# shaunlebron/blinky

Measured on AMD Instinct MI355X. Metric: warped Mpixels/s (lensmap apply), higher is better.
Workload: dtype u8; 1 GPU; 3840x2160 cube/panini f_fov 180, 64 frames/step from a resident ring of 64 distinct globes (1.80 GB, advanced every step), one lensmap; value / ms_per_step = the job with steps alternating between 2 HIP stream(s), value_one_stream = the same on one stream, roofline.kernel_ms_per_launch = the kernel alone under HIP events; 64 frames/step since r5 (r1-r4 ran 16: compare those with value_at_16_frames; ring_globes=64, parallelism=row-stripes x1, streams=2

## Files before the change

### blinky_amd/csrc/bk_api.cpp

```cpp
#include "bk_internal.h"

#include <algorithm>
#include <cstdlib>
#include <cstring>
#include <ctime>
#include <vector>

#include <dlfcn.h>

static thread_local std::string g_create_error;

static bool g_hwq_late = false;
__attribute__((constructor)) static void bk_more_hardware_queues()
{
    const char *keep = getenv("BLINKY_HIP_KEEP_HW_QUEUES");
    if (keep && *keep && *keep != '0') return;
    if (getenv("GPU_MAX_HW_QUEUES")) return;
    if (void *h = dlopen("libamdhip64.so", RTLD_NOW | RTLD_NOLOAD)) { g_hwq_late = true; (void)dlclose(h); }
    (void)setenv("GPU_MAX_HW_QUEUES", "16", 0);
}
void bk::hw_queue_note()
{
    static bool said = false;
    if (said) return;
// ... 320 lines not shown
    return BK_OK;
}

bk::DebugOptions bk::g_debug;
#if BK_DEBUG_API
extern "C" int bk_debug_set_option(const char *name, int value)
{
    if (!name) return BK_E_INVALID;
    if (!strcmp(name, "no_memcache")) bk::g_debug.no_memcache = value;
    else if (!strcmp(name, "libm_rel_log2")) bk::g_debug.libm_rel_log2 = value;
    else if (!strcmp(name, "print_model")) bk::g_debug.print_model = value;
    else if (!strcmp(name, "host_module")) bk::g_debug.host_module = value;
    else if (!strcmp(name, "no_direct_submit")) bk::g_debug.no_direct_submit = value;
    else if (!strcmp(name, "forward_careful")) bk::g_debug.forward_careful = value;
    else return BK_E_INVALID;
    return BK_OK;
}
#endif
#if BK_DEBUG_API
extern "C" int bk_debug_set_ablation(bk_ctx *ctx, int bits)
{
    if (!ctx) return BK_E_INVALID;
    ctx->apply_flags = bits;
    return BK_OK;
}
#endif

#if BK_DEBUG_API
extern "C" int bk_debug_set_tile_shape(bk_ctx *ctx, int lw)
{
    if (!ctx) return BK_E_INVALID;
    if (lw >= 600) { ctx->apply_block_cost = lw == 600 ? -1 : lw - 601; bk::coopmap_invalidate(ctx); return BK_OK; }
    if (lw >= 400) { ctx->apply_lds_kb = lw - 400; bk::coopmap_invalidate(ctx); return BK_OK; }
    if (lw >= 300) { ctx->apply_fchunk = lw - 300; return BK_OK; }
    if (lw >= 100) { ctx->apply_wgs_per_cu = lw - 100; return BK_OK; }
    if (lw != 0 && lw != 1 && lw != 2 && lw != 4) return BK_E_INVALID;
    ctx->tile_shape = lw;
    bk::coopmap_invalidate(ctx);
    return BK_OK;
}
#endif

#if BK_DEBUG_API
extern "C" int bk_debug_tile_stats(bk_ctx *ctx, int out[6])
{
    if (!ctx || !out) return BK_E_INVALID;
    if (!ctx->lensmap_valid) return ctx->fail(BK_E_STATE, "no lensmap");
    if (int r = ensure_device(ctx)) return r;
    return bk::coopmap_stats(ctx, out);
}
#endif

#if BK_DEBUG_API
extern "C" int bk_debug_traffic_model(bk_ctx *ctx, uint64_t out[8])
{
    if (!ctx || !out) return BK_E_INVALID;
    if (!ctx->lensmap_valid) return ctx->fail(BK_E_STATE, "no lensmap");
    if (int r = ensure_device(ctx)) return r;
    return bk::coopmap_traffic_model(ctx, out);
}
#endif

#if BK_DEBUG_API
extern "C" int bk_debug_band_balance(bk_ctx *ctx, uint32_t out[18])
{
    if (!ctx || !out) return BK_E_INVALID;
    if (!ctx->lensmap_valid) return ctx->fail(BK_E_STATE, "no lensmap");
    if (int r = ensure_device(ctx)) return r;
    return bk::coopmap_band_balance(ctx, out);
}
#endif

#if BK_DEBUG_API
extern "C" int bk_debug_xcd_of_workgroups(bk_ctx *ctx, int *out, int nworkgroups)
{
    if (!ctx || !out || nworkgroups < 1) return BK_E_INVALID;
    if (int r = ensure_device(ctx)) return r;
    return bk::coopmap_xcd_probe(ctx, out, nworkgroups);
}
#endif

extern "C" double bk_last_build_ms(const bk_ctx *ctx) { return ctx ? ctx->last_build_ms : 0; }


extern "C" int bk_set_lensmap(bk_ctx *ctx, const uint32_t *offsets, const uint8_t *tints)
{
    if (!ctx || !offsets) return BK_E_INVALID;
    if (!ctx->d_offsets) return ctx->fail(BK_E_STATE, "bk_set_lensmap: call bk_resize first");
    if (int r = ensure_device(ctx)) return r;
    const size_t px = (size_t)ctx->W * ctx->rows();
    BK_HIP(ctx, hipMemcpyAsync(ctx->d_offsets, offsets, px * 4, hipMemcpyHostToDevice, ctx->stream));
    if (int r = bk::launch_convert_offsets(ctx, ctx->d_offsets, px, 1)) return r;
    if (tints) BK_HIP(ctx, hipMemcpyAsync(ctx->d_tints, tints, px, hipMemcpyHostToDevice, ctx->stream));
    else BK_HIP(ctx, hipMemsetAsync(ctx->d_tints, 255, px, ctx->stream));
    if (int r = bk::subtexel_alloc(ctx)) return r;
    if (ctx->d_subtexel) BK_HIP(ctx, hipMemsetAsync(ctx->d_subtexel, 0x80, px * 2, ctx->stream));
    BK_HIP(ctx, hipStreamSynchronize(ctx->stream));
    bk::lensmap_replaced(ctx);
    return BK_OK;
}

int bk::subtexel_alloc(bk_ctx *ctx)
{
    if (!ctx->subtexel_on || ctx->d_subtexel || !ctx->map_px) return BK_OK;
    BK_HIP(ctx, hipMalloc((void **)&ctx->d_subtexel, ctx->map_px * sizeof(uint16_t)));
    return BK_OK;
// ... 940 lines not shown
```

### blinky_amd/csrc/bk_apply_coop.hip

```cpp
#include <algorithm>
#include <cmath>
#include <cstdio>
#include <cstdlib>
#include <cstring>
#include <ctime>
#include <vector>

#include "bk_internal.h"
#include "bk_resident_plan.h"

namespace bk {

constexpr int BK_PAL_BYTES = BK_MAX_PLATES * 256;
constexpr int BK_COOP_MAX_FLIPS = 4;
constexpr int BK_COOP_LDS_CAP = 65536;
constexpr uint32_t BK_COOP_MAX_CHUNKS = 4095;
constexpr uint32_t CF_ALL = 0x1, CF_NONE = 0x10;
constexpr uint32_t CF_SLOW = 0x100, CF_EMPTY = 0x200;
constexpr uint32_t BK_COOP_BINS = 65;
constexpr int BK_COOP_STATS = 208;
constexpr int BK_COOP_BLOCK_COST = 4;

enum BkAblation : int {
    BK_AB_NO_GLOBE_LOADS = 2,
// ... 21 lines not shown
constexpr int BK_KF_ALIGNED4 = 1024;
constexpr int BK_KF_ALIGNED16 = 2048;
constexpr int BK_KF_DIRECT = 1 << 27;
constexpr int BK_KF_WGMAP = 1 << 30;
static_assert((BK_RF_KERNEL_MASK & (BK_KF_ALIGNED4 | BK_KF_ALIGNED16)) == 0, "a developer bit would read as a frame alignment in the resident kernel");
static_assert((int)BK_RF_NO_STORES == (int)BK_AB_NO_STORES, "coop_gather_store reads one no-stores bit for the batch and the resident kernel");

constexpr int CS_MAX_CHUNKS = 0;
constexpr int CS_SLOW_BLOCKS = 1;
constexpr int CS_EMPTY_BLOCKS = 2;
constexpr int CS_LINES = 3;
constexpr int CS_CHUNKS = 4;
constexpr int CS_UNEVEN_BANDS = 7;
constexpr int CS_HIST_BLOCKS = 8;
constexpr int CS_HIST_LINES = CS_HIST_BLOCKS + BK_COOP_BINS;
constexpr int CS_HIST_CHUNKS = CS_HIST_LINES + BK_COOP_BINS;
static_assert(CS_HIST_CHUNKS + (int)BK_COOP_BINS <= BK_COOP_STATS, "a statistics replica holds the three histograms");

struct CoopHdr {
    uint32_t nchunks;
    uint32_t flags;
};

struct CoopMap {
    CoopHdr *d_hdr = nullptr;
    uint32_t *d_list = nullptr;
    uint16_t *d_idx = nullptr;
    bool tinted = false;
    uint32_t *d_cost = nullptr;
    uint32_t *d_order = nullptr;
    uint32_t *d_cum = nullptr;
    uint32_t *d_bands = nullptr;
    uint32_t *d_wgmap = nullptr;
    uint32_t *d_stats = nullptr;
    int blocks_x = 0, blocks_y = 0;
    int rg = 4;
    int lds_bytes = 0;
    int tuned_frames = 0;
    int single_form = 0;
    int fchunk = 0;
    bool lds_fixed = false;
    struct Tuned { int rg = 0, kb = 0, form = 0, fchunk = 0, frames = 0; } tuned[3];
    int flips = 0;
    int grown_rg = 0;
    uint32_t stats[BK_COOP_STATS] = {0};
    uint32_t *h_stats = nullptr;
    hipEvent_t stats_ready = nullptr;
    bool stats_pending = false;
    int slow_blocks = 0;
    bool valid = false;
    size_t alloc_px = 0, alloc_blocks = 0;
};

template <int RG>
__global__ __launch_bounds__(256) void coop_compile_kernel(const uint32_t *__restrict__ lmap, const uint8_t *__restrict__ tints,
                                                           int W, int rows, int blocks_x, int nblocks,
                                                           CoopHdr *__restrict__ hdr, uint32_t *__restrict__ list,
                                                           uint16_t *__restrict__ idx, int tinted,
                                                           uint32_t *__restrict__ stats, int row_stride, uint32_t *__restrict__ cost,
                                                           int block_cost)
{
    constexpr int NP = 4 * RG, N = 256 * NP;
    __shared__ uint32_t key[N];
    __shared__ uint32_t uniq[N];
    __shared__ uint32_t s_wsum[4], s_wlines[4], s_wpx[4];
    __shared__ uint32_t s_flags;
    const int lane = threadIdx.x & 63, wave = threadIdx.x >> 6;
    const bool survey = row_stride > 1;
    const int sby = blockIdx.x / blocks_x, bx = blockIdx.x - sby * blocks_x;
    const int by = sby * row_stride, blk = by * blocks_x + bx;
    constexpr int LPR = 32 / RG;
    const int oy = by * 8 * RG;
    const int ry = wave * 2 * RG + lane / LPR;
    const int x0 = bx * 128 + (lane % LPR) * 4 * RG;
    if (threadIdx.x == 0) s_flags = 0;

    uint32_t o[NP];
    uint32_t kc[NP];
    bool all_l = true, any_l = false;
    uint32_t npx = 0;
#pragma unroll
    for (int i = 0; i < NP; ++i) {
        const int row = oy + ry, x = x0 + i;
        const bool in = row < rows && x < W;
        o[i] = in ? lmap[(size_t)row * W + x] : BK_NULL_OFFSET;
        const uint32_t tn = in && tinted ? tints[(size_t)row * W + x] : 255u;
        kc[i] = o[i] == BK_NULL_OFFSET ? 0xFFFFFFFFu : ((o[i] >> 4) << 3) | (tn < (uint32_t)BK_MAX_PLATES ? tn + 1u : 0u);
        key[threadIdx.x * NP + i] = kc[i];
        all_l = all_l && o[i] != BK_NULL_OFFSET;
        any_l = any_l || o[i] != BK_NULL_OFFSET;
        npx += o[i] != BK_NULL_OFFSET ? 1u : 0u;
    }
    const bool all = __all(all_l), any = __any(any_l);
    __syncthreads();
    if (lane == 0) atomicOr(&s_flags, (all ? CF_ALL << wave : 0u) | (any ? 0u : CF_NONE << wave));

    for (int k = 2; k <= N; k <<= 1) {
        for (int j = k >> 1; j > 0; j >>= 1) {
            for (int t = threadIdx.x; t < N / 2; t += 256) {
                const int i = ((t & ~(j - 1)) << 1) | (t & (j - 1)), p = i | j;
                const uint32_t a = key[i], b = key[p];
                const bool up = (i & k) == 0;
                if ((a > b) == up) { key[i] = b; key[p] = a; }
            }
            __syncthreads();
        }
    }

    uint32_t cnt = 0, lcnt = 0;
#pragma unroll
    for (int i = 0; i < NP; ++i) {
        const int p = threadIdx.x * NP + i;
        const uint32_t v = key[p], prev = p > 0 ? key[p - 1] : 0xFFFFFFFFu;
        const bool first = v != 0xFFFFFFFFu && (p == 0 || v != prev);
        cnt += first ? 1u : 0u;
        lcnt += (first && (p == 0 || (v >> 6) != (prev >> 6))) ? 1u : 0u;
    }
    uint32_t incl = cnt, lsum = lcnt;
    for (int m = 1; m < 64; m <<= 1) {
        const uint32_t u = __shfl_up(incl, m);
        if (lane >= m) incl += u;
    }
    for (int m = 32; m >= 1; m >>= 1) { lsum += __shfl_xor(lsum, m); npx += __shfl_xor(npx, m); }
    if (lane == 63) s_wsum[wave] = incl;
    if (lane == 0) { s_wlines[wave] = lsum; s_wpx[wave] = npx; }
    __syncthreads();
    uint32_t base = incl - cnt;
    for (int w = 0; w < wave; ++w) base += s_wsum[w];
    const uint32_t nchunks = s_wsum[0] + s_wsum[1] + s_wsum[2] + s_wsum[3];
    const uint32_t lines = s_wlines[0] + s_wlines[1] + s_wlines[2] + s_wlines[3];
    const uint32_t mapped = s_wpx[0] + s_wpx[1] + s_wpx[2] + s_wpx[3];
    const bool slow = nchunks > BK_COOP_MAX_CHUNKS;
    {
        uint32_t k = base;
#pragma unroll
        for (int i = 0; i < NP; ++i) {
            const int p = threadIdx.x * NP + i;
            const uint32_t v = key[p];
            if (v != 0xFFFFFFFFu && (p == 0 || v != key[p - 1])) {
                uniq[k] = v;
                if (!slow && !survey) list[(size_t)blk * N + k] = ((v >> 3) << 4) | (v & 7u);
                ++k;
            }
        }
    }
    __syncthreads();

    if (!survey) {
#pragma unroll
    for (int r = 0; r < RG; ++r) {
        uint32_t a[4];
#pragma unroll
        for (int k = 0; k < 4; ++k) {
            const int i = r * 4 + k;
            a[k] = 0xFFFFu;
            if (o[i] != BK_NULL_OFFSET) {
                a[k] = 0;
                if (!slow) {
                    const uint32_t c = kc[i];
                    uint32_t lo = 0, hi = nchunks;
                    while (lo < hi) {
                        const uint32_t mid = (lo + hi) >> 1;
                        if (uniq[mid] < c) lo = mid + 1; else hi = mid;
                    }
                    a[k] = lo * 16u + (o[i] & 15u);
                }
            }
        }
        const size_t slab = (((size_t)blk * 4 + wave) * RG + r) * 256 + (size_t)lane * 4;
        *reinterpret_cast<uint2 *>(idx + slab) = make_uint2(a[0] | (a[1] << 16), a[2] | (a[3] << 16));
    }
    }
    if (threadIdx.x == 0) {
        const uint32_t wflags = s_flags;
        const bool any_blk = nchunks != 0;
        CoopHdr h;
        h.nchunks = slow ? 0u : nchunks;
        h.flags = wflags | (slow ? CF_SLOW : 0u) | (any_blk ? 0u : CF_EMPTY);
        if (!survey) {
            hdr[blk] = h;
            cost[blk] = !any_blk ? 0u : slow ? (uint32_t)N / 4u : lines + mapped * 5u / 512u + (uint32_t)block_cost;
        }
        uint32_t *st = stats + (blk & 63) * BK_COOP_STATS;
        if (!slow && any_blk) {
            atomicMax(&st[CS_MAX_CHUNKS], nchunks);
            const uint32_t bin = min(BK_COOP_BINS - 1u, (nchunks * 16u + 1023u) / 1024u);
            atomicAdd(&st[CS_HIST_BLOCKS + bin], 1u);
            atomicAdd(&st[CS_HIST_LINES + bin], lines);
            atomicAdd(&st[CS_HIST_CHUNKS + bin], nchunks);
            atomicAdd(&st[CS_LINES], lines);
            atomicAdd(&st[CS_CHUNKS], nchunks);
        }
        if (slow) atomicAdd(&st[CS_SLOW_BLOCKS], 1u);
        if (!any_blk) atomicAdd(&st[CS_EMPTY_BLOCKS], 1u);
    }
}

#define BK_LDS_BARRIER()                                                           \
    do {                                                                           \
        if (kflags & BK_AB_SYNCTHREADS) __syncthreads();                           \
        else asm volatile("s_waitcnt lgkmcnt(0)\n\ts_barrier" ::: "memory");       \
    } while (0)

template <int RG>
struct CoopIdx {
    uint2 iw[RG];
};
__device__ __forceinline__ uint4 bk_tint_chunk(uint4 q, uint32_t e, const uint8_t *pal_s)
{
    const uint32_t cls = e & 7u;
    if (cls) {
        const uint8_t *row = pal_s + (cls - 1u) * 256u;
        uint32_t w[4] = {q.x, q.y, q.z, q.w};
#pragma unroll
        for (int i = 0; i < 4; ++i)
            w[i] = (uint32_t)row[w[i] & 0xFFu] | ((uint32_t)row[(w[i] >> 8) & 0xFFu] << 8) | ((uint32_t)row[(w[i] >> 16) & 0xFFu] << 16) |
                   ((uint32_t)row[w[i] >> 24] << 24);
        q = make_uint4(w[0], w[1], w[2], w[3]);
    }
    return q;
}
#define BK_CHUNK_OFF(E_) (RUBIX ? (E_) & ~15u : (E_))
#define BK_CHUNK_VAL(Q_, E_) (RUBIX && !(kflags & BK_AB_NO_TINT) ? bk_tint_chunk((Q_), (E_), pal_s) : (Q_))
template <int RG>
struct CoopPrefetch {
    uint2 h;
    uint32_t c[4];
// ... 1100 lines not shown
    if (int r = coop_stats_wait(ctx, cm)) return r;
    const int nb = cm->blocks_x * cm->blocks_y;
    std::vector<uint32_t> cum((size_t)nb);
    BK_HIP(ctx, hipMemcpyAsync(out, cm->d_bands, 9 * sizeof(uint32_t), hipMemcpyDeviceToHost, ctx->stream));
    BK_HIP(ctx, hipMemcpyAsync(cum.data(), cm->d_cum, (size_t)nb * sizeof(uint32_t), hipMemcpyDeviceToHost, ctx->stream));
    BK_HIP(ctx, hipStreamSynchronize(ctx->stream));
    out[9] = cm->stats[CS_UNEVEN_BANDS] ? 1u : 0u;
    for (int k = 0; k < 8; ++k) {
        const uint32_t a = out[k], b = out[k + 1];
        out[10 + k] = b > a ? cum[b - 1] - (a ? cum[a - 1] : 0u) : 0u;
    }
    return BK_OK;
}

__global__ __launch_bounds__(256) void coop_row_cost_kernel(const uint32_t *__restrict__ cost, int blocks_x, int block_rows, int rows,
                                                            uint32_t *__restrict__ out)
{
    const int y = blockIdx.x * 256 + threadIdx.x;
    if (y >= rows) return;
    const int by = y / block_rows, here = min(block_rows, rows - by * block_rows);
    uint32_t s = 0;
    for (int bx = 0; bx < blocks_x; ++bx) s += cost[by * blocks_x + bx];
    out[y] = (s * 16u + (uint32_t)here / 2u) / (uint32_t)here + 16u;
}

int coopmap_row_costs(bk_ctx *ctx, uint32_t *rows_out)
{
    const int tuning = ctx->blockmap_tuning;
    const bool had_map = ctx->coopmap && ctx->coopmap->valid;
    ctx->blockmap_tuning = 0;
    const int r = ensure_coopmap(ctx);
    ctx->blockmap_tuning = tuning;
    if (r) return r;
    CoopMap *cm = ctx->coopmap;
    if (!had_map && tuning) cm->valid = false;
    if (ctx->rows() > 0) {
        hipLaunchKernelGGL(coop_row_cost_kernel, dim3((unsigned)((ctx->rows() + 255) / 256)), dim3(256), 0, ctx->stream,
                           cm->d_cost, cm->blocks_x, 8 * cm->rg, ctx->rows(), rows_out);
        BK_HIP(ctx, hipGetLastError());
    }
    return BK_OK;
}

int coopmap_stats(bk_ctx *ctx, int out[6])
{
    if (int r = ensure_coopmap(ctx)) return r;
    CoopMap *cm = ctx->coopmap;
    if (int r = coop_stats_wait(ctx, cm)) return r;
    out[0] = cm->blocks_x * cm->blocks_y; out[1] = cm->slow_blocks; out[2] = (int)cm->stats[CS_EMPTY_BLOCKS]; out[3] = cm->lds_bytes;
    out[4] = 8 * cm->rg + 1000 * 128; out[5] = (int)cm->stats[CS_LINES];
    return BK_OK;
}

#include "bk_apply_rgba.inc"
#include "bk_apply_rgba_fb.inc"
#include "bk_apply_resident.inc"
#include "bk_apply_rgba_mip.inc"

}
```

### blinky_amd/csrc/bk_internal.h

```cpp
#pragma once

#include <hip/hip_runtime.h>

#include <cstdarg>
#include <cstdint>
#include <cstdio>
#include <functional>
#include <string>
#include <vector>

#include "../../include/blinky_hip.h"
#ifndef BK_DEBUG_API
#define BK_DEBUG_API 0
#endif
#if BK_DEBUG_API
#include "../../include/blinky_hip_debug.h"
#endif
#include "bk_build_params.h"

namespace bk {

struct DebugOptions { int no_memcache = 0, libm_rel_log2 = 0, print_model = 0, host_module = 0, no_direct_submit = 0, forward_careful = 0; };
extern DebugOptions g_debug;

// ... 158 lines not shown
    }
    int rows() const { return row1 - row0; }
    size_t plate_bytes() const { return (size_t)gp * ph; }
    size_t globe_stride() const { return (size_t)BK_MAX_PLATES * gp * ph; }
    size_t plate_tiles() const { return (size_t)(gp >> 4) * (ph >> 3); }
    const int *fp_summary(int plate) const { return reinterpret_cast<const int *>(h_fp + fp_words) + 5 * plate; }
};

#define BK_HIP(ctx, expr)                                                               \
    do {                                                                                \
        hipError_t e_ = (expr);                                                         \
        if (e_ != hipSuccess)                                                           \
            return (ctx)->fail(BK_E_HIP, "%s failed: %s", #expr, hipGetErrorString(e_)); \
    } while (0)

namespace bk {

int launch_apply(bk_ctx *ctx, int frame0, int nframes, uint8_t *dst_first_owned_row, int dst_pitch,
                 size_t frame_stride, int rubix_on);
int launch_mask(bk_ctx *ctx);
int launch_fill_lcg(bk_ctx *ctx, uint8_t *plate_dst, uint32_t seed);
int launch_convert_offsets(bk_ctx *ctx, uint32_t *buf, size_t n, int to_device);
int launch_plate_retile(bk_ctx *ctx, uint8_t *plate_tiled, int to_tiled, uint8_t *rowmajor = nullptr);
int launch_plate_rgba_retile(bk_ctx *ctx, uint8_t *plane0, const uint8_t *src_dev, size_t src_pitch);
int launch_footprint(bk_ctx *ctx);
inline void footprint_invalidate(bk_ctx *ctx) { ctx->footprint_valid = false; }
int subtexel_alloc(bk_ctx *ctx);
void footprint_free(bk_ctx *ctx);
int launch_plate_rgba_retile_footprint(bk_ctx *ctx, int plate, uint8_t *plane0, const uint8_t *src_dev, size_t src_pitch);
int launch_scatter32(bk_ctx *ctx, uint32_t *dst, const uint32_t *h_idx, const uint32_t *h_val, size_t n);
int launch_scatter8(bk_ctx *ctx, uint8_t *dst, const uint32_t *h_idx, const uint8_t *h_val, size_t n);
int launch_scatter16(bk_ctx *ctx, uint16_t *dst, const uint32_t *h_idx, const uint16_t *h_val, size_t n);
int launch_truncate_scan(bk_ctx *ctx, unsigned int bad_key, int display_out[BK_MAX_PLATES]);
void coopmap_invalidate(bk_ctx *ctx);
inline void lod_invalidate(bk_ctx *ctx) { ctx->lod_state = 0; }
inline void lensmap_edited(bk_ctx *ctx) { ctx->spans_valid = false; coopmap_invalidate(ctx); footprint_invalidate(ctx); lod_invalidate(ctx); }
inline void lensmap_dropped(bk_ctx *ctx) { ctx->lensmap_valid = ctx->subtexel_valid = false; lensmap_edited(ctx); }
inline void lensmap_replaced(bk_ctx *ctx) { ctx->lensmap_valid = true; ctx->subtexel_valid = ctx->d_subtexel != nullptr; lensmap_edited(ctx); }
int launch_apply_coop(bk_ctx *ctx, int frame0, int nframes, uint8_t *dst_first_owned_row, int dst_pitch,
                      size_t frame_stride, int rubix_on);
int launch_apply_rgba(bk_ctx *ctx, int globe0, int nframes, uint8_t *dst_first_owned_row, int dst_pitch, size_t frame_stride,
                      const uint8_t *d_lut = nullptr, bool ss2 = false);
enum FbMode { FB_NEAREST, FB_SS2, FB_BILINEAR, FB_BILINEAR_SEAMS };
int launch_apply_rgba_fb(bk_ctx *ctx, const void *const plates[BK_MAX_PLATES], const int pitches[BK_MAX_PLATES], uint8_t *dst, int dst_pitch,
                         const uint8_t *d_lut, FbMode mode);
#define BK_MIP_TABLE_BYTES 256
inline int mip_level_count(int ps) { int n = 0; for (int s = ps; s >= 1; s = (s + 1) / 2) { ++n; if (s == 1) break; } return n; }
int launch_mip_pyramid(bk_ctx *ctx, const void *const plates[BK_MAX_PLATES], const int pitches[BK_MAX_PLATES]);
int launch_lod(bk_ctx *ctx);
int launch_apply_rgba_fb_trilinear(bk_ctx *ctx, const void *const plates[BK_MAX_PLATES], const int pitches[BK_MAX_PLATES], uint8_t *dst, int dst_pitch,
                                   const uint8_t *d_lut);
int coopmap_stats(bk_ctx *ctx, int out[6]);
int coopmap_traffic_model(bk_ctx *ctx, uint64_t out[8]);
int coopmap_xcd_probe(bk_ctx *ctx, int *out, int nwg);
int coopmap_band_balance(bk_ctx *ctx, uint32_t out[18]);
int coopmap_row_costs(bk_ctx *ctx, uint32_t *rows_out);
}
int bk_row_costs_device(bk_ctx *ctx, uint32_t *cost_dev);
namespace bk {
void coopmap_free(CoopMap *);
int resident_begin(bk_ctx *ctx, int rubix_on, double idle_ms);
int resident_submit(bk_ctx *ctx, int frame, uint8_t *dst_first_owned_row, int dst_pitch, uint64_t *ticket);
int resident_wait(bk_ctx *ctx, uint64_t ticket, double *gpu_us);
int resident_stop(bk_ctx *ctx);
void resident_free(bk_ctx *ctx);
int resident_info(bk_ctx *ctx, int out[12]);
inline void resident_quiesce(bk_ctx *ctx) { if (ctx->resident) (void)resident_stop(ctx); }
bool resident_leaves_room(bk_ctx *ctx);
void hw_queue_note();
void host_parallel(size_t parts, const std::function<void(size_t)> &job);
bool resident_running(bk_ctx *ctx);

void lensprogram_free(LensProgram *);
int build_module_ready(bk_ctx *ctx);
void empty_context(bk_ctx *ctx);
inline void seam_drop(bk_ctx *ctx) { ctx->seam_valid = ctx->seam_user = ctx->d_seam_current = false; }
int seam_table_ready(bk_ctx *ctx, const char *who);
int seam_table_compute(bk_ctx *ctx, std::vector<uint32_t> &out);

}
```

### blinky_amd/ffi.py

```python
import ctypes as C
import os

import numpy as np

try:
    import torch
except ImportError:
    torch = None

LIB_PATH = os.environ.get("BLINKY_HIP_LIB") or os.path.join(os.path.dirname(os.path.abspath(__file__)), "libblinkyhip.so")
if not os.path.exists(LIB_PATH):
    raise ImportError(
        f"{LIB_PATH} is missing: build it with `python -c 'import __graft_entry__ as g; g.build()'` "
        "(or `make -C blinky_amd/csrc`).  There is no CPU fallback."
    )
lib = C.CDLL(LIB_PATH)

MAX_PLATES = 6
MIP_MAX_LEVELS = 16
NULL_OFFSET = 0xFFFFFFFF
DEVICE_NONE = -2
OK = 0
PENDING = 1
MAP_NONE, MAP_INVERSE, MAP_FORWARD = 0, 1, 2
# ... 54 lines not shown
    "bk_upload_plate_rgba_footprint_device": (_i, [_vp, _i, _i, _vp, _i]),
    "bk_apply_rgba_device": (_i, [_vp, _i, _i, _vp, _i, _sz, _i, _i]),
    "bk_apply_rgba_tinted_device": (_i, [_vp, _i, _i, _vp, _i, _sz, _i, _i, _vp]),
    "bk_apply_rgba_ss2_device": (_i, [_vp, _i, _i, _vp, _i, _sz, _i, _i, _vp]),
    "bk_apply_rgba_fb_device": (_i, [_vp, C.POINTER(_vp), C.POINTER(_i), _vp, _i, _i, _i, _vp, _i]),
    "bk_apply_rgba_fb_bilinear_device": (_i, [_vp, C.POINTER(_vp), C.POINTER(_i), _vp, _i, _i, _i, _vp]),
    "bk_apply_rgba_fb_bilinear_seams_device": (_i, [_vp, C.POINTER(_vp), C.POINTER(_i), _vp, _i, _i, _i, _vp]),
    "bk_apply_rgba_fb_trilinear_device": (_i, [_vp, C.POINTER(_vp), C.POINTER(_i), _vp, _i, _i, _i, _vp, _i]),
    "bk_mip_info": (_i, [_vp, C.POINTER(_i), C.POINTER(_i)]),
    "bk_read_mip_level": (_i, [_vp, _i, _i, _vp, _i]),
    "bk_set_lod_bias": (_i, [_vp, _i]),
    "bk_read_lod": (_i, [_vp, _vp]),
    "bk_set_lensmap_lod": (_i, [_vp, _vp]),
    "bk_read_seam_table": (_i, [_vp, _vp]),
    "bk_set_seam_table": (_i, [_vp, _vp]),
    "bk_debug_fb_decode_check": (C.c_longlong, [_i, _i]),
    "bk_debug_mip_pyramid": (_i, [_vp, C.POINTER(_vp), C.POINTER(_i)]),
    "bk_globe_device_ptr": (_vp, [_vp, _i]),
    "bk_fill_plate_lcg": (_i, [_vp, _i, _i, C.c_uint32]),
    "bk_apply": (_i, [_vp, _i, _vp, _i, _i, _i, _i, _vp]),
    "bk_apply_device": (_i, [_vp, _i, _i, _vp, _i, _sz, _i, _i, _i, _vp]),
    "bk_apply_begin": (_i, [_vp, _i, _i, _vp]),
    "bk_apply_resident_begin": (_i, [_vp, _i, _vp, _d]),
    "bk_apply_resident_submit": (_i, [_vp, _i, _vp, _i, _i, _i, C.POINTER(C.c_uint64)]),
    "bk_apply_resident_submit_batch": (_i, [_vp, _i, _i, _vp, _i, _sz, _i, _i, C.POINTER(C.c_uint64)]),
    "bk_apply_resident_wait": (_i, [_vp, C.c_uint64, C.POINTER(_d)]),
    "bk_apply_resident_end": (_i, [_vp]),
    "bk_apply_resident_info": (_i, [_vp, C.POINTER(_i)]),
    "bk_apply_end": (_i, [_vp, _vp, _i, _i, _i]),
    "bk_create_palmap": (None, [_vp, _vp]),
    "bk_create_tintmap_rgba": (None, [_vp, _vp]),
    "bk_get_size": (_i, [_vp] + [C.POINTER(_i)] * 5),
    "bk_version": (C.c_char_p, []),
    "bk_set_apply_variant": (_i, [_vp, _i]),
    "bk_set_resident_share": (_i, [_vp, _i, _i, _i]),
    "bk_set_resident_apply": (_i, [_vp, _i]),
    "bk_multi_set_resident_apply": (_i, [_vp, _i]),
    "bk_set_blockmap_tuning": (_i, [_vp, _i]),
    "bk_set_host_compile": (_i, [_i]),
    "bk_host_module_ready": (_i, [_vp, _i]),
    "bk_debug_module_from_cache": (_i, [_vp]),
    "bk_debug_forward_tiles": (_i, [_vp, C.POINTER(_i), C.POINTER(_i)]),
    "bk_debug_set_option": (_i, [C.c_char_p, _i]),
    "bk_debug_build_breakdown": (_i, [_vp, C.POINTER(_d)]),
    "bk_multi_lensmap_valid": (_i, [_vp]),
    "bk_last_build_ms": (_d, [_vp]),
    "bk_globe_pitch": (_i, [_vp]),
    "bk_globe_rows": (_i, [_vp]),
    "bk_globe_texel_offset": (C.c_uint32, [_vp, _i, _i, _i]),
    "bk_download_plate": (_i, [_vp, _i, _i, _vp, _i]),
    "bk_save_plate": (_i, [_vp, _i, _i, _i, _vp, _i]),
    "bk_debug_tile_stats": (_i, [_vp, C.POINTER(_i)]),
    "bk_debug_traffic_model": (_i, [_vp, C.POINTER(C.c_uint64)]),
    "bk_debug_band_balance": (_i, [_vp, C.POINTER(C.c_uint32)]),
    "bk_debug_stream_mix": (_i, [_vp, _sz, _i, _i, C.POINTER(_d)]),
    "bk_debug_fnv1a64": (_i, [_vp, _sz, C.POINTER(C.c_uint64)]),
    "bk_debug_host_build": (_i, [_vp, _i, _vp, _vp, C.POINTER(_i), C.POINTER(_d)]),
    "bk_debug_host_build_subtexel": (_i, [_vp, _i, _vp, _vp, _vp, C.POINTER(_i), C.POINTER(_d)]),
    "bk_debug_resident_latency": (_i, [_vp, _i, _vp, _i, _i, C.POINTER(_d), C.POINTER(_d)]),
    "bk_debug_build_params": (_i, [_vp, _vp, _sz, C.POINTER(_sz)]),
    "bk_debug_host_entries": (_i, [_vp, _vp, _sz, _vp, _vp]),
    "bk_debug_host_corners": (_i, [_vp, _vp, _sz, _vp, _vp, _vp]),
    "bk_debug_set_forward_corners": (_i, [_vp, _vp, _vp, _sz]),
    "bk_debug_xcd_of_workgroups": (_i, [_vp, C.POINTER(_i), _i]),
    "bk_debug_set_ablation": (_i, [_vp, _i]),
    "bk_debug_set_tile_shape": (_i, [_vp, _i]),
    "bk_debug_kernel_source": (_i, [_vp, C.c_char_p, _sz, C.POINTER(_sz), _i]),
    "bk_debug_eval": (_i, [_vp, _i, C.POINTER(_d), _i, C.POINTER(_d), C.POINTER(_i)]),
    "bk_script_console": (C.c_char_p, [_vp]),
    "bk_set_host_math": (_i, [_vp, _i]),
    "bk_debug_eval_device": (_i, [_vp, _i, _vp, _i, _i, _vp, _vp]),
    "bk_debug_eval_device_bounds": (_i, [_vp, _i, _vp, _i, _i, _vp, _vp, _vp, _vp]),
    "bk_dev_alloc": (_vp, [_vp, _sz]),
    "bk_dev_free": (None, [_vp, _vp]),
    "bk_dev_read": (_i, [_vp, _vp, _vp, _sz]),
    "bk_comm_unique_id": (_i, [_vp]),
    "bk_comm_create": (_vp, [_vp, _i, _i, _vp]),
    "bk_comm_destroy": (None, [_vp]),
    "bk_comm_last_error": (C.c_char_p, [_vp]),
    "bk_comm_stripe": (_i, [_vp, _i, C.POINTER(_i), C.POINTER(_i)]),
    "bk_comm_restripe": (_i, [_vp]),
    "bk_comm_rebalance": (_i, [_vp]),
    "bk_debug_stripe_bounds": (_i, [C.POINTER(C.c_uint32), _i, _i, _i, C.POINTER(_i)]),
    "bk_debug_row_costs": (_i, [_vp, C.POINTER(C.c_uint32)]),
    "bk_multi_rebalance": (_i, [_vp, C.POINTER(_i)]),
    "bk_comm_or_display": (_i, [_vp, C.POINTER(_i)]),
    "bk_comm_gather": (_i, [_vp, _vp, _i, _i, _vp, _sz, _i]),
    "bk_comm_exchange_rotating": (_i, [_vp, _vp, _i, _vp, _sz, _i]),
    "bk_comm_wait": (_i, [_vp, _i]),
    "bk_comm_synchronize": (_i, [_vp]),
    "bk_create_multi": (_vp, [_i, C.POINTER(_i)]),
    "bk_destroy_multi": (None, [_vp]),
    "bk_multi_last_error": (C.c_char_p, [_vp]),
    "bk_multi_size": (_i, [_vp]),
    "bk_multi_ctx": (_vp, [_vp, _i]),
    "bk_multi_comm": (_vp, [_vp, _i]),
    "bk_multi_uses_rccl": (_i, [_vp]),
    "bk_multi_load_globe": (_i, [_vp, C.c_char_p, _sz, C.c_char_p]),
    "bk_multi_load_lens": (_i, [_vp, C.c_char_p, _sz, C.c_char_p]),
    "bk_multi_clear_lens": (_i, [_vp]),
    "bk_multi_clear_globe": (_i, [_vp]),
    "bk_multi_resize": (_i, [_vp, _i, _i]),
    "bk_multi_set_frames": (_i, [_vp, _i]),
    "bk_multi_set_zoom": (_i, [_vp, _i, _i]),
    "bk_multi_set_rubixgrid": (_i, [_vp, _i, _d, _d]),
    "bk_multi_upload_plate": (_i, [_vp, _i, _i, _vp, _i]),
# ... 386 lines not shown
        table = np.ascontiguousarray(table, dtype=np.uint32)
        if table.size != MAX_PLATES * 4 * (ps + 2):
            raise ValueError(f"table must be uint32 [{MAX_PLATES}][4][{ps + 2}], not {table.shape}")
        self._chk(lib.bk_set_seam_table(self._h, _ptr(table)))

    def resident_begin(self, rubix_on=False, pal=None, idle_ms=0.0):
        if pal is not None:
            pal = np.ascontiguousarray(pal, dtype=np.uint8)
        self._chk(lib.bk_apply_resident_begin(self._h, int(rubix_on), _ptr(pal), float(idle_ms)))

    def resident_submit(self, dst_ptr, pitch, frame=0, x0=0, y0=0):
        t = C.c_uint64(0)
        self._chk(lib.bk_apply_resident_submit(self._h, frame, dst_ptr, pitch, x0, y0, C.byref(t)))
        return t.value

    def resident_submit_batch(self, dst_ptr, pitch, frame_stride, frame0=0, nframes=1, x0=0, y0=0):
        t = C.c_uint64(0)
        self._chk(lib.bk_apply_resident_submit_batch(self._h, frame0, nframes, dst_ptr, pitch, frame_stride, x0, y0, C.byref(t)))
        return t.value

    def resident_wait(self, ticket):
        us = _d(0)
        self._chk(lib.bk_apply_resident_wait(self._h, ticket, C.byref(us)))
        return us.value

    def resident_end(self):
        self._chk(lib.bk_apply_resident_end(self._h))

    def resident_latency(self, dst_ptr, pitch, frames=200, globes=1):
        h, d = _d(), _d()
        self._chk(lib.bk_debug_resident_latency(self._h, frames, dst_ptr, pitch, globes, C.byref(h), C.byref(d)))
        return h.value, d.value

    def resident_info(self):
        out = (_i * 12)()
        self._chk(lib.bk_apply_resident_info(self._h, out))
        return dict(running=bool(out[0]), workgroups=out[1], blocks_in_registers=out[2], chunks_per_thread=out[3], block_h=out[4],
                    per_cu=out[5], launches=out[6], pending=out[7], streamed=(out[8], out[9], out[10]), laggard=out[11] // 10000, laggards=out[11] % 10000)

    def host_module_ready(self, wait=False):
        return bool(lib.bk_host_module_ready(self._h, int(wait)))

    def set_blockmap_tuning(self, measured):
        self._chk(lib.bk_set_blockmap_tuning(self._h, int(measured)))

    def set_ablation(self, bits):
        self._chk(lib.bk_debug_set_ablation(self._h, bits))

    def tile_stats(self):
        out = (_i * 6)()
        self._chk(lib.bk_debug_tile_stats(self._h, out))
        return dict(tiles=out[0], slow=out[1], empty=out[2], lds_bytes_per_wave=out[3], tile_h=out[4], lines=out[5])

    def row_costs(self):
        _, H = self.size()[:2]
        out = np.zeros(H, np.uint32)
        self._chk(lib.bk_debug_row_costs(self._h, out.ctypes.data_as(C.POINTER(C.c_uint32))))
        return out

    def build_params(self):
        need = _sz()
        self._chk(lib.bk_debug_build_params(self._h, None, 0, C.byref(need)))
        buf = C.create_string_buffer(need.value)
        self._chk(lib.bk_debug_build_params(self._h, buf, need.value, None))
        return buf

    def host_entries(self, ids):
        ids = np.ascontiguousarray(ids, dtype=np.uint32)
        off = np.empty(len(ids), np.uint32)
        tin = np.empty(len(ids), np.uint8)
        self._chk(lib.bk_debug_host_entries(self._h, _ptr(ids), len(ids), _ptr(off), _ptr(tin)))
        return off, tin

    def host_corners(self, ids):
        ids = np.ascontiguousarray(ids, dtype=np.uint32)
        sx = np.empty(len(ids), np.int32)
        sy = np.empty(len(ids), np.int32)
        ok = np.empty(len(ids), np.uint8)
        self._chk(lib.bk_debug_host_corners(self._h, _ptr(ids), len(ids), _ptr(sx), _ptr(sy), _ptr(ok)))
        return sx, sy, ok

    def set_forward_corners(self, xy=None, ok=None):
        if xy is None or ok is None:
            self._chk(lib.bk_debug_set_forward_corners(self._h, None, None, 0))
            return
        xy = np.ascontiguousarray(xy, dtype=np.int32)
        ok = np.ascontiguousarray(ok, dtype=np.uint8)
        if xy.size != 2 * ok.size:
            raise ValueError("set_forward_corners: xy must hold two coordinates per corner")
        self._chk(lib.bk_debug_set_forward_corners(self._h, _ptr(xy), _ptr(ok), ok.size))

    def xcd_of_workgroups(self, n):
        out = (_i * n)()
        self._chk(lib.bk_debug_xcd_of_workgroups(self._h, out, n))
        return list(out)

    def traffic_model(self):
        out = (C.c_uint64 * 8)()
        self._chk(lib.bk_debug_traffic_model(self._h, out))
        return dict(unique_globe_lines=out[0], staged_lines=out[1], staged_chunks=out[2], blockmap_bytes_per_visit=out[3],
                    mapped_pixels=out[4], frames_per_visit=out[5], blocks=out[6], block_height=out[7])

    def stream_mix(self, nbytes, period, writes):
        out = _d()
        self._chk(lib.bk_debug_stream_mix(self._h, nbytes, period, writes, C.byref(out)))
        return out.value
# ... 288 lines not shown
```

### include/blinky_hip_debug.h

```cpp
#ifndef BLINKY_HIP_DEBUG_H
#define BLINKY_HIP_DEBUG_H

#include "blinky_hip.h"

#ifdef __cplusplus
extern "C" {
#endif

int         bk_debug_set_option(const char *name, int value);
int         bk_debug_module_from_cache(const bk_ctx *ctx);
int         bk_debug_forward_tiles(bk_ctx *ctx, int *taken, int *total);
int         bk_debug_set_ablation(bk_ctx *ctx, int bits);
int         bk_debug_tile_stats(bk_ctx *ctx, int out[6]);
int         bk_debug_traffic_model(bk_ctx *ctx, uint64_t out[8]);
int         bk_debug_band_balance(bk_ctx *ctx, uint32_t out[18]);
int         bk_debug_stream_mix(bk_ctx *ctx, size_t bytes, int period, int writes, double *gbps);
int         bk_debug_host_build(bk_ctx *ctx, int mode, uint32_t *offsets, uint8_t *tints, int display_out[BK_MAX_PLATES], double *scale_out);
int         bk_debug_host_build_subtexel(bk_ctx *ctx, int mode, uint32_t *offsets, uint8_t *tints, uint16_t *sub, int display_out[BK_MAX_PLATES],
                                         double *scale_out);
int         bk_debug_fnv1a64(const void *host, size_t bytes, uint64_t *out);
int         bk_debug_resident_latency(bk_ctx *ctx, int frames, void *dst_dev, int dst_pitch, int globes, double *host_us, double *device_us);
int         bk_debug_xcd_of_workgroups(bk_ctx *ctx, int *out, int nworkgroups);
int         bk_debug_set_tile_shape(bk_ctx *ctx, int lw);
int         bk_debug_kernel_source(bk_ctx *ctx, char *buf, size_t cap, size_t *needed, int compile);
int         bk_debug_build_params(bk_ctx *ctx, void *out, size_t cap, size_t *needed);
int         bk_debug_host_entries(bk_ctx *ctx, const uint32_t *ids, size_t n, uint32_t *offsets, uint8_t *tints);
int         bk_debug_host_corners(bk_ctx *ctx, const uint32_t *ids, size_t n, int32_t *sx, int32_t *sy, uint8_t *ok);
int         bk_debug_set_forward_corners(bk_ctx *ctx, const int32_t *xy, const uint8_t *ok, size_t ncorners);
int         bk_debug_eval(bk_ctx *ctx, int which, const double *args, int nargs, double out[8], int *nout);
int         bk_debug_eval_device(bk_ctx *ctx, int which, const double *args, int nargs, int n, double *out, int *nout);
int         bk_debug_eval_device_bounds(bk_ctx *ctx, int which, const double *args, int nargs, int n, double *out, double *bound, int *flag,
                                        int *nout);
int         bk_debug_build_breakdown(const bk_ctx *ctx, double out[6]);
int         bk_debug_stripe_bounds(const uint32_t *row_cost, int H, int W, int nranks, int *bounds_out);
int         bk_debug_row_costs(bk_ctx *ctx, uint32_t *host_out);
long long   bk_debug_fb_decode_check(int gp, int ph);
int         bk_debug_mip_pyramid(bk_ctx *ctx, const void *const plates_dev[BK_MAX_PLATES], const int plate_pitch_bytes[BK_MAX_PLATES]);

#ifdef __cplusplus
}
#endif
#endif
```

Before: 2.656 million Mpixels/s.

## Dedupe coop block chunks with an LDS hash table before sorting only unique keys

The one-time lensmap compile kernel now inserts chunk keys into a shared-memory hash table with atomicCAS to remove duplicates, then bitonic-sorts only the unique keys (padded to a power of two) using multi-stage register sorting with bank-padded indexing. Previously it sorted all pixels' keys. This reduces the compile kernel's shared-memory footprint and sort work. It also adds a debug readback API for the block map. The compile kernel runs once per lensmap, so the per-frame apply throughput being measured is unlikely to change.

```diff
diff --git a/blinky_amd/csrc/bk_api.cpp b/blinky_amd/csrc/bk_api.cpp
--- a/blinky_amd/csrc/bk_api.cpp
+++ b/blinky_amd/csrc/bk_api.cpp
@@ -396,6 +396,16 @@
 #endif
 
 #if BK_DEBUG_API
+extern "C" int bk_debug_read_blockmap(bk_ctx *ctx, int info[4], uint32_t *hdr, uint32_t *list, size_t list_entries, uint16_t *idx)
+{
+    if (!ctx || !info) return BK_E_INVALID;
+    if (!ctx->lensmap_valid) return ctx->fail(BK_E_STATE, "no lensmap");
+    if (int r = ensure_device(ctx)) return r;
+    return bk::coopmap_read(ctx, info, hdr, list, list_entries, idx);
+}
+#endif
+
+#if BK_DEBUG_API
 extern "C" int bk_debug_traffic_model(bk_ctx *ctx, uint64_t out[8])
 {
     if (!ctx || !out) return BK_E_INVALID;
diff --git a/blinky_amd/csrc/bk_apply_coop.hip b/blinky_amd/csrc/bk_apply_coop.hip
--- a/blinky_amd/csrc/bk_apply_coop.hip
+++ b/blinky_amd/csrc/bk_apply_coop.hip
@@ -97,6 +97,38 @@
     size_t alloc_px = 0, alloc_blocks = 0;
 };
 
+template <int BITS>
+__device__ __forceinline__ uint32_t coop_key_home(uint32_t key) { return (key * 0x9E3779B1u) >> (32 - BITS); }
+
+__device__ __forceinline__ uint32_t coop_at(uint32_t x) { return x + (x >> 4); }
+
+template <int G>
+__device__ __forceinline__ void coop_bitonic_stages(uint32_t *tab, uint32_t M, uint32_t k, int b)
+{
+    constexpr int E = 1 << G;
+    const uint32_t low = (1u << b) - 1u;
+    for (uint32_t g = threadIdx.x; g < (M >> G); g += 256) {
+        const uint32_t base = ((g & ~low) << G) | (g & low);
+        const bool up = (base & k) == 0;
+        uint32_t e[E];
+#pragma unroll
+        for (int i = 0; i < E; ++i) e[i] = tab[coop_at(base + ((uint32_t)i << b))];
+#pragma unroll
+        for (int s = G - 1; s >= 0; --s) {
+#pragma unroll
+            for (int i = 0; i < E; ++i) {
+                if (i & (1 << s)) continue;
+                const uint32_t lo = e[i], hi = e[i | (1 << s)];
+                const bool swap = (lo > hi) == up;
+                e[i] = swap ? hi : lo;
+                e[i | (1 << s)] = swap ? lo : hi;
+            }
+        }
+#pragma unroll
+        for (int i = 0; i < E; ++i) tab[coop_at(base + ((uint32_t)i << b))] = e[i];
+    }
+}
+
 template <int RG>
 __global__ __launch_bounds__(256) void coop_compile_kernel(const uint32_t *__restrict__ lmap, const uint8_t *__restrict__ tints,
                                                            int W, int rows, int blocks_x, int nblocks,
@@ -106,10 +138,12 @@
                                                            int block_cost)
 {
     constexpr int NP = 4 * RG, N = 256 * NP;
-    __shared__ uint32_t key[N];
-    __shared__ uint32_t uniq[N];
-    __shared__ uint32_t s_wsum[4], s_wlines[4], s_wpx[4];
-    __shared__ uint32_t s_flags;
+    constexpr int BITS = RG == 4 ? 13 : RG == 2 ? 12 : 11, SLOTS = 1 << BITS, SPT = SLOTS / 256;
+    static_assert(SLOTS == 2 * N, "the dedupe table has two slots per pixel");
+    constexpr uint32_t NONE = 0xFFFFFFFFu;
+    __shared__ uint32_t tab[SLOTS];
+    static_assert(N + N / 16 <= SLOTS - 16, "the padded unique list stays clear of the scratch words");
+    uint32_t *const s_wsum = tab + SLOTS - 16, *const s_wflags = s_wsum + 4, *const s_wpx = s_wsum + 8, *const s_wlines = s_wsum + 12;
     const int lane = threadIdx.x & 63, wave = threadIdx.x >> 6;
     const bool survey = row_stride > 1;
     const int sby = blockIdx.x / blocks_x, bx = blockIdx.x - sby * blocks_x;
@@ -118,80 +152,103 @@
     const int oy = by * 8 * RG;
     const int ry = wave * 2 * RG + lane / LPR;
     const int x0 = bx * 128 + (lane % LPR) * 4 * RG;
-    if (threadIdx.x == 0) s_flags = 0;
-
-    uint32_t o[NP];
+#pragma unroll
+    for (int j = 0; j < SPT; ++j) tab[j * 256 + threadIdx.x] = NONE;
+
     uint32_t kc[NP];
+    uint64_t byte_in_chunk = 0;
     bool all_l = true, any_l = false;
     uint32_t npx = 0;
 #pragma unroll
     for (int i = 0; i < NP; ++i) {
         const int row = oy + ry, x = x0 + i;
         const bool in = row < rows && x < W;
-        o[i] = in ? lmap[(size_t)row * W + x] : BK_NULL_OFFSET;
+        const uint32_t o = in ? lmap[(size_t)row * W + x] : BK_NULL_OFFSET;
         const uint32_t tn = in && tinted ? tints[(size_t)row * W + x] : 255u;
-        kc[i] = o[i] == BK_NULL_OFFSET ? 0xFFFFFFFFu : ((o[i] >> 4) << 3) | (tn < (uint32_t)BK_MAX_PLATES ? tn + 1u : 0u);
-        key[threadIdx.x * NP + i] = kc[i];
-        all_l = all_l && o[i] != BK_NULL_OFFSET;
-        any_l = any_l || o[i] != BK_NULL_OFFSET;
-        npx += o[i] != BK_NULL_OFFSET ? 1u : 0u;
+        kc[i] = o == BK_NULL_OFFSET ? NONE : ((o >> 4) << 3) | (tn < (uint32_t)BK_MAX_PLATES ? tn + 1u : 0u);
+        byte_in_chunk |= (uint64_t)(o & 15u) << (4 * i);
+        all_l = all_l && o != BK_NULL_OFFSET;
+        any_l = any_l || o != BK_NULL_OFFSET;
+        npx += o != BK_NULL_OFFSET ? 1u : 0u;
     }
     const bool all = __all(all_l), any = __any(any_l);
     __syncthreads();
-    if (lane == 0) atomicOr(&s_flags, (all ? CF_ALL << wave : 0u) | (any ? 0u : CF_NONE << wave));
-
-    for (int k = 2; k <= N; k <<= 1) {
-        for (int j = k >> 1; j > 0; j >>= 1) {
-            for (int t = threadIdx.x; t < N / 2; t += 256) {
-                const int i = ((t & ~(j - 1)) << 1) | (t & (j - 1)), p = i | j;
-                const uint32_t a = key[i], b = key[p];
-                const bool up = (i & k) == 0;
-                if ((a > b) == up) { key[i] = b; key[p] = a; }
-            }
-            __syncthreads();
-        }
-    }
-
-    uint32_t cnt = 0, lcnt = 0;
+
 #pragma unroll
     for (int i = 0; i < NP; ++i) {
-        const int p = threadIdx.x * NP + i;
-        const uint32_t v = key[p], prev = p > 0 ? key[p - 1] : 0xFFFFFFFFu;
-        const bool first = v != 0xFFFFFFFFu && (p == 0 || v != prev);
-        cnt += first ? 1u : 0u;
-        lcnt += (first && (p == 0 || (v >> 6) != (prev >> 6))) ? 1u : 0u;
-    }
-    uint32_t incl = cnt, lsum = lcnt;
+        if (kc[i] != NONE && (i == 0 || kc[i] != kc[i > 0 ? i - 1 : 0])) {
+            uint32_t s = coop_key_home<BITS>(kc[i]);
+            for (;;) {
+                const uint32_t old = atomicCAS(&tab[s], NONE, kc[i]);
+                if (old == NONE || old == kc[i]) break;
+                s = (s + 1u) & (uint32_t)(SLOTS - 1);
+            }
+        }
+    }
+    __syncthreads();
+
+    uint32_t v[SPT];
+    uint32_t cnt = 0;
+#pragma unroll
+    for (int j = 0; j < SPT; ++j) {
+        v[j] = tab[j * 256 + threadIdx.x];
+        cnt += v[j] != NONE ? 1u : 0u;
+    }
+    uint32_t incl = cnt;
     for (int m = 1; m < 64; m <<= 1) {
         const uint32_t u = __shfl_up(incl, m);
         if (lane >= m) incl += u;
     }
-    for (int m = 32; m >= 1; m >>= 1) { lsum += __shfl_xor(lsum, m); npx += __shfl_xor(npx, m); }
+    for (int m = 32; m >= 1; m >>= 1) npx += __shfl_xor(npx, m);
+    __syncthreads();
     if (lane == 63) s_wsum[wave] = incl;
-    if (lane == 0) { s_wlines[wave] = lsum; s_wpx[wave] = npx; }
+    if (lane == 0) { s_wflags[wave] = (all ? CF_ALL << wave : 0u) | (any ? 0u : CF_NONE << wave); s_wpx[wave] = npx; }
     __syncthreads();
     uint32_t base = incl - cnt;
     for (int w = 0; w < wave; ++w) base += s_wsum[w];
     const uint32_t nchunks = s_wsum[0] + s_wsum[1] + s_wsum[2] + s_wsum[3];
-    const uint32_t lines = s_wlines[0] + s_wlines[1] + s_wlines[2] + s_wlines[3];
+    const uint32_t wflags = s_wflags[0] | s_wflags[1] | s_wflags[2] | s_wflags[3];
     const uint32_t mapped = s_wpx[0] + s_wpx[1] + s_wpx[2] + s_wpx[3];
     const bool slow = nchunks > BK_COOP_MAX_CHUNKS;
+    uint32_t M = 2;
+    while (M < nchunks) M <<= 1;
     {
         uint32_t k = base;
 #pragma unroll
-        for (int i = 0; i < NP; ++i) {
-            const int p = threadIdx.x * NP + i;
-            const uint32_t v = key[p];
-            if (v != 0xFFFFFFFFu && (p == 0 || v != key[p - 1])) {
-                uniq[k] = v;
-                if (!slow && !survey) list[(size_t)blk * N + k] = ((v >> 3) << 4) | (v & 7u);
-                ++k;
-            }
-        }
+        for (int j = 0; j < SPT; ++j)
+            if (v[j] != NONE) tab[coop_at(k++)] = v[j];
+        for (uint32_t p = nchunks + threadIdx.x; p < M; p += 256) tab[coop_at(p)] = NONE;
     }
     __syncthreads();
 
+    constexpr int MAXG = RG == 1 ? 2 : 3;
+    uint32_t lcnt = 0;
+    if (!slow) {
+        int lk = 1;
+        for (uint32_t k = 2; k <= M; k <<= 1, ++lk) {
+            for (int top = lk; top > 0;) {
+                const int g = top < MAXG ? top : MAXG;
+                top -= g;
+                if (MAXG >= 3 && g == 3) coop_bitonic_stages<MAXG >= 3 ? 3 : 1>(tab, M, k, top);
+                else if (g == 2) coop_bitonic_stages<2>(tab, M, k, top);
+                else coop_bitonic_stages<1>(tab, M, k, top);
+                __syncthreads();
+            }
+        }
+        for (uint32_t p = threadIdx.x; p < nchunks; p += 256) {
+            const uint32_t c = tab[coop_at(p)];
+            lcnt += (p == 0 || (c >> 6) != (tab[coop_at(p - 1)] >> 6)) ? 1u : 0u;
+            if (!survey) list[(size_t)blk * N + p] = ((c >> 3) << 4) | (c & 7u);
+        }
+    }
+    for (int m = 32; m >= 1; m >>= 1) lcnt += __shfl_xor(lcnt, m);
+    if (lane == 0) s_wlines[wave] = lcnt;
+    __syncthreads();
+    const uint32_t lines = s_wlines[0] + s_wlines[1] + s_wlines[2] + s_wlines[3];
+    const uint32_t *const uniq = tab;
+
     if (!survey) {
+    uint32_t slot = 0;
 #pragma unroll
     for (int r = 0; r < RG; ++r) {
         uint32_t a[4];
@@ -199,16 +256,19 @@
         for (int k = 0; k < 4; ++k) {
             const int i = r * 4 + k;
             a[k] = 0xFFFFu;
-            if (o[i] != BK_NULL_OFFSET) {
+            if (kc[i] != NONE) {
                 a[k] = 0;
                 if (!slow) {
-                    const uint32_t c = kc[i];
-                    uint32_t lo = 0, hi = nchunks;
-                    while (lo < hi) {
-                        const uint32_t mid = (lo + hi) >> 1;
-                        if (uniq[mid] < c) lo = mid + 1; else hi = mid;
+                    if (i == 0 || kc[i] != kc[i > 0 ? i - 1 : 0]) {
+                        const uint32_t c = kc[i];
+                        uint32_t lo = 0, hi = nchunks;
+                        while (lo < hi) {
+                            const uint32_t mid = (lo + hi) >> 1;
+                            if (uniq[coop_at(mid)] < c) lo = mid + 1; else hi = mid;
+                        }
+                        slot = lo;
                     }
-                    a[k] = lo * 16u + (o[i] & 15u);
+                    a[k] = slot * 16u + ((uint32_t)(byte_in_chunk >> (4 * i)) & 15u);
                 }
             }
         }
@@ -217,7 +277,6 @@
     }
     }
     if (threadIdx.x == 0) {
-        const uint32_t wflags = s_flags;
         const bool any_blk = nchunks != 0;
         CoopHdr h;
         h.nchunks = slow ? 0u : nchunks;
@@ -1424,6 +1483,33 @@
     return BK_OK;
 }
 
+int coopmap_read(bk_ctx *ctx, int info[4], uint32_t *hdr_out, uint32_t *list_out, size_t list_cap, uint16_t *idx_out)
+{
+    if (int r = ensure_coopmap(ctx)) return r;
+    const CoopMap *cm = ctx->coopmap;
+    BK_HIP(ctx, hipStreamSynchronize(ctx->stream));
+    const size_t nb = (size_t)cm->blocks_x * cm->blocks_y, N = (size_t)1024 * cm->rg;
+    std::vector<CoopHdr> hdr(nb);
+    BK_HIP(ctx, hipMemcpy(hdr.data(), cm->d_hdr, nb * sizeof(CoopHdr), hipMemcpyDeviceToHost));
+    size_t entries = 0;
+    for (const CoopHdr &h : hdr) entries += h.nchunks;
+    info[0] = cm->rg; info[1] = cm->blocks_x; info[2] = cm->blocks_y; info[3] = (int)entries;
+    if (hdr_out) memcpy(hdr_out, hdr.data(), nb * sizeof(CoopHdr));
+    if (list_out) {
+        if (list_cap < entries) return ctx->fail(BK_E_INVALID, "bk_debug_read_blockmap: the list buffer is too small");
+        std::vector<uint32_t> all(nb * N);
+        BK_HIP(ctx, hipMemcpy(all.data(), cm->d_list, nb * N * sizeof(uint32_t), hipMemcpyDeviceToHost));
+        size_t at = 0;
+        for (size_t b = 0; b < nb; ++b) {
+            if (hdr[b].nchunks > N) return ctx->fail(BK_E_STATE, "bk_debug_read_blockmap: a block lists more chunks than it has pixels");
+            memcpy(list_out + at, all.data() + b * N, hdr[b].nchunks * sizeof(uint32_t));
+            at += hdr[b].nchunks;
+        }
+    }
+    if (idx_out) BK_HIP(ctx, hipMemcpy(idx_out, cm->d_idx, nb * N * sizeof(uint16_t), hipMemcpyDeviceToHost));
+    return BK_OK;
+}
+
 #include "bk_apply_rgba.inc"
 #include "bk_apply_rgba_fb.inc"
 #include "bk_apply_resident.inc"
diff --git a/blinky_amd/csrc/bk_internal.h b/blinky_amd/csrc/bk_internal.h
--- a/blinky_amd/csrc/bk_internal.h
+++ b/blinky_amd/csrc/bk_internal.h
@@ -234,6 +234,7 @@
                                    const uint8_t *d_lut);
 int coopmap_stats(bk_ctx *ctx, int out[6]);
 int coopmap_traffic_model(bk_ctx *ctx, uint64_t out[8]);
+int coopmap_read(bk_ctx *ctx, int info[4], uint32_t *hdr_out, uint32_t *list_out, size_t list_cap, uint16_t *idx_out);
 int coopmap_xcd_probe(bk_ctx *ctx, int *out, int nwg);
 int coopmap_band_balance(bk_ctx *ctx, uint32_t out[18]);
 int coopmap_row_costs(bk_ctx *ctx, uint32_t *rows_out);
diff --git a/blinky_amd/ffi.py b/blinky_amd/ffi.py
--- a/blinky_amd/ffi.py
+++ b/blinky_amd/ffi.py
@@ -130,6 +130,7 @@
     "bk_save_plate": (_i, [_vp, _i, _i, _i, _vp, _i]),
     "bk_debug_tile_stats": (_i, [_vp, C.POINTER(_i)]),
     "bk_debug_traffic_model": (_i, [_vp, C.POINTER(C.c_uint64)]),
+    "bk_debug_read_blockmap": (_i, [_vp, C.POINTER(_i), _vp, _vp, _sz, _vp]),
     "bk_debug_band_balance": (_i, [_vp, C.POINTER(C.c_uint32)]),
     "bk_debug_stream_mix": (_i, [_vp, _sz, _i, _i, C.POINTER(_d)]),
     "bk_debug_fnv1a64": (_i, [_vp, _sz, C.POINTER(C.c_uint64)]),
@@ -622,6 +623,17 @@
         self._chk(lib.bk_debug_tile_stats(self._h, out))
         return dict(tiles=out[0], slow=out[1], empty=out[2], lds_bytes_per_wave=out[3], tile_h=out[4], lines=out[5])
 
+    def read_blockmap(self):
+        info = (_i * 4)()
+        self._chk(lib.bk_debug_read_blockmap(self._h, info, None, None, 0, None))
+        rg, bx, by, entries = info[0], info[1], info[2], info[3]
+        hdr = np.empty((bx * by, 2), np.uint32)
+        flat = np.empty(entries, np.uint32)
+        idx = np.empty((bx * by, 4, rg, 64, 4), np.uint16)
+        self._chk(lib.bk_debug_read_blockmap(self._h, info, _ptr(hdr), _ptr(flat), entries, _ptr(idx)))
+        lists = np.split(flat, np.cumsum(hdr[:, 0].astype(np.int64))[:-1]) if bx * by else []
+        return dict(rg=rg, blocks_x=bx, blocks_y=by, hdr=hdr, lists=lists, idx=idx)
+
     def row_costs(self):
         _, H = self.size()[:2]
         out = np.zeros(H, np.uint32)
diff --git a/include/blinky_hip_debug.h b/include/blinky_hip_debug.h
--- a/include/blinky_hip_debug.h
+++ b/include/blinky_hip_debug.h
@@ -12,6 +12,7 @@
 int         bk_debug_forward_tiles(bk_ctx *ctx, int *taken, int *total);
 int         bk_debug_set_ablation(bk_ctx *ctx, int bits);
 int         bk_debug_tile_stats(bk_ctx *ctx, int out[6]);
+int         bk_debug_read_blockmap(bk_ctx *ctx, int info[4], uint32_t *hdr, uint32_t *list, size_t list_entries, uint16_t *idx);
 int         bk_debug_traffic_model(bk_ctx *ctx, uint64_t out[8]);
 int         bk_debug_band_balance(bk_ctx *ctx, uint32_t out[18]);
 int         bk_debug_stream_mix(bk_ctx *ctx, size_t bytes, int period, int writes, double *gbps);
```

Result: no change. 2.654 million Mpixels/s (-0.1%).
